# JuliaGaussianProcesses/AugmentedGPLikelihoods.jl

Measured on AMD Instinct MI355X. Metric: CAVI sweeps/sec (N obs, M inducing) + max |Δnat-param| vs CPU ref, higher is better.
Workload: dtype f32 via f16 hi/lo split operands (3 f16 MFMA products per f32 product, f32 accumulate, f64 reductions and M x M update)

## Files before the change

augmentedgplikelihoods.jl_amd/csrc/agpl_syrk.hip:

```cpp
#include <cstdlib>

#include "agpl_common.h"

namespace {

typedef _Float16 h8 __attribute__((ext_vector_type(8)));
typedef float f32x4 __attribute__((ext_vector_type(4)));
typedef unsigned u32x4 __attribute__((ext_vector_type(4)));

constexpr int BS = 128;
constexpr int kPanel = 256;
constexpr int kStagePts = 32;
constexpr uint32_t kImageMagic = 0x41474951u;

struct AccImageHeader {
    uint32_t magic;
    int32_t scale_exp;
    float max_abs;
    uint32_t reserved;
    int64_t N;
    int32_t M;
    int32_t pad[57];
};
static_assert(sizeof(AccImageHeader) == 256, "header size");

__device__ __forceinline__ f32x4 mfma32(h8 a, h8 b, f32x4 c) {
    return __builtin_amdgcn_mfma_f32_16x16x32_f16(a, b, c, 0, 0, 0);
}

#define AGPL_E_SPLIT2(x0_, s0_, x1_, s1_, H_, L_)                                                              \
    do {                                                                                                       \
        asm("v_fma_mixlo_f16 %0, %1, %2, 0" : "=v"(H_) : "v"(x0_), "v"(s0_));                                  \
        asm("v_fma_mixhi_f16 %0, %1, %2, 0" : "+v"(H_) : "v"(x1_), "v"(s1_));                                  \
        asm("v_fma_mixlo_f16 %0, %1, %2, -%3 op_sel_hi:[0,0,1]" : "=v"(L_) : "v"(x0_), "v"(s0_), "v"(H_));     \
        asm("v_fma_mixhi_f16 %0, %1, %2, -%3 op_sel:[0,0,1] op_sel_hi:[0,0,1]"                                 \
            : "+v"(L_)                                                                                         \
            : "v"(x1_), "v"(s1_), "v"(H_));                                                                    \
    } while (0)
#define AGPL_E_GFMA(acc_, b_, x_) asm volatile("v_fmac_f32 %0, %1, %2" : "+v"(acc_) : "v"(b_), "v"(x_))
#define AGPL_Q_JOIN2(H_, L_, x0_, x1_)                                                                         \
    do {                                                                                                       \
        asm("v_fma_mix_f32 %0, %1, 1.0, %2 op_sel_hi:[1,0,1]" : "=v"(x0_) : "v"(H_), "v"(L_));                 \
        asm("v_fma_mix_f32 %0, %1, 1.0, %2 op_sel:[1,0,1] op_sel_hi:[1,0,1]" : "=v"(x1_) : "v"(H_), "v"(L_));  \
    } while (0)

__global__ __launch_bounds__(256) void absmax_kernel(int64_t n4, int ntail, const float4 *__restrict__ x, unsigned *__restrict__ out) {
    unsigned m = 0u;
    for (int64_t i = (int64_t)blockIdx.x * blockDim.x + threadIdx.x; i < n4; i += (int64_t)gridDim.x * blockDim.x) {
        const float4 v = x[i];
        m = max(m, __float_as_uint(v.x) & 0x7FFFFFFFu);
        m = max(m, __float_as_uint(v.y) & 0x7FFFFFFFu);
        m = max(m, __float_as_uint(v.z) & 0x7FFFFFFFu);
        m = max(m, __float_as_uint(v.w) & 0x7FFFFFFFu);
    }
    if (blockIdx.x == 0 && (int)threadIdx.x < ntail)
        m = max(m, __float_as_uint(reinterpret_cast<const float *>(x)[4 * n4 + threadIdx.x]) & 0x7FFFFFFFu);
#pragma unroll
    for (int o = 32; o > 0; o >>= 1) m = max(m, (unsigned)__shfl_xor((int)m, o));
    if ((threadIdx.x & 63) == 0 && m) atomicMax(out, m);
}

__global__ __launch_bounds__(256) void find_bad_kernel(int64_t n, const float *__restrict__ x, float limit,
                                                       unsigned long long *__restrict__ out) {
    for (int64_t i = (int64_t)blockIdx.x * blockDim.x + threadIdx.x; i < n; i += (int64_t)gridDim.x * blockDim.x) {
        const float a = fabsf(x[i]);
        if (!(a < limit)) atomicMin(out, (unsigned long long)i);
    }
}

__global__ __launch_bounds__(256) void accumulate_image_kernel(int64_t N, int M, int Msrc, int64_t nps, float scale, int scale_exp,
                                                               float max_abs, const float *__restrict__ Phi,
                                                               unsigned char *__restrict__ image) {
    __shared__ float tile[16][BS + 1];
    const int nb = M / BS;
    if (blockIdx.x == 0 && threadIdx.x == 0) {
        AccImageHeader *h = reinterpret_cast<AccImageHeader *>(image);
        h->magic = kImageMagic;
        h->scale_exp = scale_exp;
        h->max_abs = max_abs;
        h->reserved = 0;
        h->N = N;
        h->M = M;
    }
    h8 *blocks = reinterpret_cast<h8 *>(image + sizeof(AccImageHeader));
    const int64_t nblk = nps * nb;
    for (int64_t blk = blockIdx.x; blk < nblk; blk += gridDim.x) {
        const int64_t ps = blk / nb;
        const int fb = (int)(blk - ps * nb);
        {
            const int pt = threadIdx.x >> 4, f0 = (threadIdx.x & 15) * 8;
            const int64_t n = ps * 16 + pt;
            float4 a = {0.f, 0.f, 0.f, 0.f}, b = a;
            if (n < N) {
                const int fg = fb * BS + f0;
                const float *src = Phi + n * (int64_t)Msrc + fg;
                if (!(Msrc & 3) && fg + 8 <= Msrc) {
                    a = *reinterpret_cast<const float4 *>(src);
                    b = *reinterpret_cast<const float4 *>(src + 4);
                } else {
                    float t[8];
#pragma unroll
                    for (int j = 0; j < 8; ++j) t[j] = fg + j < Msrc ? src[j] : 0.f;
                    a = float4{t[0], t[1], t[2], t[3]};
                    b = float4{t[4], t[5], t[6], t[7]};
                }
            }
            float *d = &tile[pt][f0];
            d[0] = a.x; d[1] = a.y; d[2] = a.z; d[3] = a.w;
            d[4] = b.x; d[5] = b.y; d[6] = b.z; d[7] = b.w;
        }
        __syncthreads();
        const int plane = threadIdx.x >> 7, row = threadIdx.x & 127;
        h8 hi, lo;
#pragma unroll
        for (int j = 0; j < 8; ++j) {
            const float x = tile[plane * 8 + j][row] * scale;
            const _Float16 a = (_Float16)x;
            hi[j] = a;
            lo[j] = (_Float16)(x - (float)a);
        }
        blocks[(blk * 2 + 0) * 256 + threadIdx.x] = hi;
        blocks[(blk * 2 + 1) * 256 + threadIdx.x] = lo;
        __syncthreads();
    }
}

__global__ __launch_bounds__(256) void acc_prep_kernel(int64_t N, int64_t Npad, int L, const float *__restrict__ gamma,
                                                        const float *__restrict__ beta, float *__restrict__ gb,
                                                        unsigned *__restrict__ scal) {
    __shared__ unsigned red[2][4];
    const int64_t total = (int64_t)L * Npad;
    unsigned m = 0u, bd = 0u;
    for (int64_t i = (int64_t)blockIdx.x * blockDim.x + threadIdx.x; i < total; i += (int64_t)gridDim.x * blockDim.x) {
        const int64_t l = i / Npad, n = i - l * Npad;
        const bool in = n < N;
        const float gv = in ? gamma[l * N + n] : 0.f;
        const unsigned gbits = __float_as_uint(gv), ab = gbits & 0x7FFFFFFFu;
        const bool bad = ab >= 0x7F800000u || ((gbits >> 31) && ab != 0u);
        if (bad) bd = max(bd, (unsigned)min((int64_t)0x7FFFFFFE, l * N + n) + 1u);
        m = max(m, bad ? 0u : ab);
        float *rec = gb + (l * (Npad / 32) + n / 32) * 64 + (n & 31);
        rec[0] = gv;
        rec[32] = in ? beta[l * N + n] : 0.f;
    }
#pragma unroll
    for (int o = 32; o > 0; o >>= 1) {
        m = max(m, (unsigned)__shfl_xor((int)m, o));
        bd = max(bd, (unsigned)__shfl_xor((int)bd, o));
    }
    if ((threadIdx.x & 63) == 0) {
        red[0][threadIdx.x >> 6] = m;
        red[1][threadIdx.x >> 6] = bd;
    }
    __syncthreads();
    if (threadIdx.x == 0) {
        for (int w = 1; w < 4; ++w) {
            m = max(m, red[0][w]);
            bd = max(bd, red[1][w]);
        }
        if (m) atomicMax(scal, m);
        if (bd) atomicMax(scal + 1, bd);
    }
}

__device__ __forceinline__ int acc_scale_exp(unsigned gmax) {
    int eB = gmax ? 126 - (int)(gmax >> 23) : 0;
    return eB < -60 ? -60 : (eB > 60 ? 60 : eB);
}

#ifdef AGPL_QTRACE
__device__ unsigned long long g_qtrace[64 * 16 * 8];
constexpr bool kTrace = true;
#else
constexpr bool kTrace = false;
#endif

#ifdef AGPL_SYRK_L2PROBE
#define AGPL_PROBE_T(t_) ((t_) & 3)
#else
#define AGPL_PROBE_T(t_) (t_)
#endif
#ifdef AGPL_SYRK_NODMA
#define AGPL_PROBE_LOAD(t_) ((t_) < 3)
#else
#define AGPL_PROBE_LOAD(t_) true
#endif
#ifndef AGPL_S_PRE
#define AGPL_S_PRE 3
#endif
constexpr int kStepBytes = 32768;
constexpr int kRing = 4;
constexpr int kRecBytes = 256;
constexpr int kStripLds = kRing * kStepBytes + 8 * kRing * kRecBytes;

template <bool DIAG>
__device__ __forceinline__ void syrk_strip_body(unsigned char *smem_raw, int64_t N, int64_t Npad, int M, int nsplit, int chunk, int nbig, int small, int l,
                                                int s, int I, int J, const unsigned char *__restrict__ image,
                                                const float *__restrict__ gb_all, const unsigned *__restrict__ scal,
                                                float *__restrict__ slabG, float *__restrict__ slabg) {
    typedef __attribute__((address_space(3))) void lds_void;
    const int lane = threadIdx.x & 63;
    const int wave = __builtin_amdgcn_readfirstlane(threadIdx.x >> 6);
    const int nb = M / BS;
    const int c = DIAG ? ((wave & 4) ? 7 - (wave & 3) : (wave & 3)) : wave;
    const int i0 = DIAG ? 2 * c : 0;
    const AccImageHeader *hdr = reinterpret_cast<const AccImageHeader *>(image);
    const h8 *blocks = reinterpret_cast<const h8 *>(image + sizeof(AccImageHeader));
    const int eA = hdr->scale_exp;
    const int eB = acc_scale_exp(scal[0]);
    const float sB = __uint_as_float((unsigned)(127 + eB) << 23);

    int64_t nbeg, nend;
    agpl_slice_range(s, chunk, nbig, small, N, nbeg, nend);
    const int nstep = (int)((nend - nbeg + kStagePts - 1) / kStagePts);
    const int64_t ps0 = nbeg / 16;
    const int64_t slice_pitch = (int64_t)nb * 2 * 256;

    int ln = lane;
    asm volatile("" : "+v"(ln));
    const int kg = ln >> 4, lr = ln & 15;
    const int rbS = (wave >> 2) & 1, qd = wave & 3;
    const h8 *a_src = blocks + ((ps0 * nb + 2 * I + rbS) * 2) * 256 + qd * 64 + lane;
    const int a_dst = rbS * 2 * 4096 + qd * 1024;
    const int R0 = 32 * c + lr;
    const h8 *b_src = blocks + (((ps0 + (kg >> 1)) * nb + 2 * J + (R0 >> 7)) * 2) * 256 + (kg & 1) * 128 + (R0 & 127);
    const float *gb_src = gb_all + ((int64_t)l * (Npad / 32) + nbeg / 32) * 64 + lane;
    float *gbuf = reinterpret_cast<float *>(smem_raw + kRing * kStepBytes + wave * kRing * kRecBytes);

    f32x4 acc[16][2];
#pragma unroll
    for (int i = 0; i < 16; ++i) acc[i][0] = acc[i][1] = f32x4{0.f, 0.f, 0.f, 0.f};
    float gacc0 = 0.f, gacc1 = 0.f;
    u32x4 rh0 = {0, 0, 0, 0}, rl0 = rh0, rh1 = rh0, rl1 = rh0;
    h8 bh0, bl0, bh1, bl1;

#define AGPL_S_DMA(t_, k_)                     \
    do {                                                                                                        \
        unsigned char *d_ = smem_raw + ((t_) & (kRing - 1)) * kStepBytes + ((k_) >> 1) * 16384 + a_dst + ((k_) & 1) * 4096; \
        const h8 *src_ = a_src + (int64_t)(2 * AGPL_PROBE_T(t_) + ((k_) >> 1)) * slice_pitch + ((k_) & 1) * 256; \
        if (AGPL_PROBE_LOAD(t_)) __builtin_amdgcn_global_load_lds(src_, (lds_void *)d_, 16, 0, 0);              \
    } while (0)
#define AGPL_S_DMAG(t_)                                                                                         \
    if (AGPL_PROBE_LOAD(t_))                                                                                    \
    __builtin_amdgcn_global_load_lds(gb_src + (int64_t)(t_) * 64, (lds_void *)(gbuf + ((t_) & (kRing - 1)) * 64), 4, 0, 0)
#define AGPL_S_LOADB(t_)                                                                                        \
    do {                                                                                                        \
        const h8 *src_ = b_src + (int64_t)(2 * AGPL_PROBE_T(t_)) * slice_pitch;                                 \
        const h8 *srcl_ = src_ + 256;  \
        if (AGPL_PROBE_LOAD(t_))                                                                                \
        asm volatile("global_load_dwordx4 %0, %4, off\n\tglobal_load_dwordx4 %1, %5, off\n\t"                   \
                     "global_load_dwordx4 %2, %4, off offset:256\n\tglobal_load_dwordx4 %3, %5, off offset:256"  \
                     : "+v"(rh0), "+v"(rl0), "+v"(rh1), "+v"(rl1)                                               \
                     : "v"(src_), "v"(srcl_)                                                                    \
                     : "memory");                                                                               \
    } while (0)
#define AGPL_S_CVT(RH_, RL_, g0_, g1_, b0_, b1_, GA_)                                                           \
    do {                                                                                                        \
        float x0_, x1_;                                                                                         \
        AGPL_Q_JOIN2(RH_, RL_, x0_, x1_);                                                                       \
        if (DIAG) {                                                                                             \
            AGPL_E_GFMA(GA_, b0_, x0_);                                                                         \
            AGPL_E_GFMA(GA_, b1_, x1_);                                                                         \
        }                                                                                                       \
        AGPL_E_SPLIT2(x0_, g0_, x1_, g1_, RH_, RL_);                                                            \
    } while (0)
#define AGPL_S_CVTQ(q_, tt_, keepf_)                                                                            \
    do {                                                                                                        \
        const float *gq_ = gbuf + ((tt_) & (kRing - 1)) * 64 + 8 * kg + 4 * ((q_) & 1);                         \
        float4 g4_ = *reinterpret_cast<const float4 *>(gq_);                                                    \
        g4_.x *= sB, g4_.y *= sB, g4_.z *= sB, g4_.w *= sB;                                                     \
        float4 b4_ = {0.f, 0.f, 0.f, 0.f};                                                                      \
        if (DIAG) {                                                                                             \
            b4_ = *reinterpret_cast<const float4 *>(gq_ + 32);                                                  \
            if (!(keepf_)) b4_ = float4{0.f, 0.f, 0.f, 0.f};                                                    \
        }                                                                                                       \
        if ((q_) == 0) {                                                                                        \
            AGPL_S_CVT(rh0.x, rl0.x, g4_.x, g4_.y, b4_.x, b4_.y, gacc0);                                        \
            AGPL_S_CVT(rh0.y, rl0.y, g4_.z, g4_.w, b4_.z, b4_.w, gacc0);                                        \
            AGPL_S_CVT(rh1.x, rl1.x, g4_.x, g4_.y, b4_.x, b4_.y, gacc1);                                        \
            AGPL_S_CVT(rh1.y, rl1.y, g4_.z, g4_.w, b4_.z, b4_.w, gacc1);                                        \
        } else {                                                                                                \
            AGPL_S_CVT(rh0.z, rl0.z, g4_.x, g4_.y, b4_.x, b4_.y, gacc0);                                        \
            AGPL_S_CVT(rh0.w, rl0.w, g4_.z, g4_.w, b4_.z, b4_.w, gacc0);                                        \
            AGPL_S_CVT(rh1.z, rl1.z, g4_.x, g4_.y, b4_.x, b4_.y, gacc1);                                        \
            AGPL_S_CVT(rh1.w, rl1.w, g4_.z, g4_.w, b4_.z, b4_.w, gacc1);                                        \
        }                                                                                                       \
    } while (0)
#define AGPL_S_TAKEB()                       \
    do {                                                                                                        \
        bh0 = __builtin_bit_cast(h8, rh0);                                                                      \
        bl0 = __builtin_bit_cast(h8, rl0);                                                                      \
        bh1 = __builtin_bit_cast(h8, rh1);                                                                      \
        bl1 = __builtin_bit_cast(h8, rl1);                                                                      \
    } while (0)

    const int fa = (kg >> 1) * 1024 + (kg & 1) * 128 + lr;
#define AGPL_S_AOFF(i_) (fa + ((i_) >> 3) * 512 + ((i_) & 7) * 16)
#define AGPL_S_LDSB(t_)                                                                                         \
    do {                                                                                                        \
        const u32x4 *sn_ = reinterpret_cast<const u32x4 *>(smem_raw + ((t_) & (kRing - 1)) * kStepBytes);       \
        rh0 = sn_[AGPL_S_AOFF(2 * c)];                                                                          \
        rl0 = sn_[256 + AGPL_S_AOFF(2 * c)];                                                                    \
        rh1 = sn_[AGPL_S_AOFF(2 * c + 1)];                                                                      \
        rl1 = sn_[256 + AGPL_S_AOFF(2 * c + 1)];                                                                \
    } while (0)

#pragma unroll
    for (int t = 0; t < 3; ++t)
        if (t < nstep) {
            AGPL_S_DMAG(t);
            AGPL_S_DMA(t, 0);
            AGPL_S_DMA(t, 1);
            AGPL_S_DMA(t, 2);
            AGPL_S_DMA(t, 3);
        }
    if (!DIAG) AGPL_S_LOADB(0);
    asm volatile("s_waitcnt vmcnt(0)" ::: "memory");
    __builtin_amdgcn_sched_barrier(0);
    if (DIAG) {
        __builtin_amdgcn_s_barrier();
        AGPL_S_LDSB(0);
    }
    AGPL_S_CVTQ(0, 0, true);
    AGPL_S_CVTQ(1, 0, true);
    AGPL_S_TAKEB();
    if (!DIAG) AGPL_S_LOADB(nstep > 1 ? 1 : 0);

    [[maybe_unused]] unsigned long long q0 = 0, q1 = 0, qw = 0, qa = 0, qb = 0, qr0 = 0;
    if (kTrace) {
        q0 = __builtin_amdgcn_s_memtime();
        qr0 = __builtin_amdgcn_s_memrealtime();
    }
    for (int t = 0; t < nstep; ++t) {
        if (kTrace) qa = __builtin_amdgcn_s_memtime();
        if (!DIAG) __builtin_amdgcn_s_barrier();
        if (kTrace && !DIAG) qw += __builtin_amdgcn_s_memtime() - qa;
        const bool more = t + 1 < nstep;
        const int tl = t + 2 < nstep ? t + 2 : nstep - 1;
        const h8 *st = reinterpret_cast<const h8 *>(smem_raw + (t & (kRing - 1)) * kStepBytes);
#define AGPL_S_HOOK(h_)                                                                                         \
    do {                                                                                                        \
        if (!DIAG) {                                                                                            \
            if ((h_) < 4 && t + 3 < nstep) {                                                                    \
                if ((h_) == 0) AGPL_S_DMAG(t + 3);                                                              \
                AGPL_S_DMA(t + 3, h_);                                                                          \
            }                                                                                                   \
            if ((h_) == 5) {  \
                __builtin_amdgcn_sched_barrier(0);                                                              \
                if (t + 3 < nstep) asm volatile("s_waitcnt vmcnt(5)" ::: "memory");                             \
                else asm volatile("s_waitcnt vmcnt(0)" ::: "memory");                                           \
                __builtin_amdgcn_sched_barrier(0);                                                              \
            }                                                                                                   \
            if ((h_) == 6) AGPL_S_CVTQ(0, t + 1, more);                                                         \
            if ((h_) == 8) AGPL_S_CVTQ(1, t + 1, more);                                                         \
        } else {                                                                                                \
             \
             \
             \
                 \
            if ((h_) == 7) {                                                                                    \
                __builtin_amdgcn_sched_barrier(0);                                                              \
                if (kTrace) qb = __builtin_amdgcn_s_memtime();                                                  \
                if (t + 2 < nstep) asm volatile("s_waitcnt vmcnt(5)" ::: "memory");                             \
                else asm volatile("s_waitcnt vmcnt(0)" ::: "memory");                                           \
                if (kTrace) q1 += __builtin_amdgcn_s_memtime() - qb;                                            \
                if (kTrace) qb = __builtin_amdgcn_s_memtime();                                                  \
                __builtin_amdgcn_s_barrier();                                                                   \
                if (kTrace) qw += __builtin_amdgcn_s_memtime() - qb;                                            \
                __builtin_amdgcn_sched_barrier(0);                                                              \
                AGPL_S_LDSB(more ? t + 1 : t);                 \
            }                                                                                                   \
            if ((h_) >= 8 && (h_) < 12 && t + 3 < nstep) {                                                      \
                if ((h_) == 8) AGPL_S_DMAG(t + 3);                                                              \
                AGPL_S_DMA(t + 3, (h_) - 8);                                                                    \
            }                                                                                                   \
            if ((h_) == 9) AGPL_S_CVTQ(0, t + 1, more);                                                         \
            if ((h_) == 11) AGPL_S_CVTQ(1, t + 1, more);                                                        \
        }                                                                                                       \
    } while (0)
        h8 nbh0, nbl0, nbh1, nbl1;
        constexpr int kPre = AGPL_S_PRE;
        h8 af[kPre + 1][2];
#pragma unroll
        for (int j = 0; j < kPre; ++j) {
            af[j][0] = st[AGPL_S_AOFF(j)];
            af[j][1] = st[256 + AGPL_S_AOFF(j)];
        }
#pragma unroll
        for (int i = 0; i < 16; ++i) {
            if (i + kPre < 16) {
                af[(i + kPre) % (kPre + 1)][0] = st[AGPL_S_AOFF(i + kPre)];
                af[(i + kPre) % (kPre + 1)][1] = st[256 + AGPL_S_AOFF(i + kPre)];
            }
            if (!DIAG || i >= i0) {
                const h8 ahc = af[i % (kPre + 1)][0], alc = af[i % (kPre + 1)][1];
                acc[i][0] = mfma32(ahc, bh0, acc[i][0]);
                acc[i][1] = mfma32(ahc, bh1, acc[i][1]);
                acc[i][0] = mfma32(ahc, bl0, acc[i][0]);
                acc[i][1] = mfma32(ahc, bl1, acc[i][1]);
                acc[i][0] = mfma32(alc, bh0, acc[i][0]);
                acc[i][1] = mfma32(alc, bh1, acc[i][1]);
            }
            AGPL_S_HOOK(i);
            if (i == (DIAG ? 12 : 10)) {
                nbh0 = __builtin_bit_cast(h8, rh0);
                nbl0 = __builtin_bit_cast(h8, rl0);
                nbh1 = __builtin_bit_cast(h8, rh1);
                nbl1 = __builtin_bit_cast(h8, rl1);
                if (!DIAG) AGPL_S_LOADB(tl);
            }
        }
#undef AGPL_S_HOOK
        bh0 = nbh0;
        bl0 = nbl0;
        bh1 = nbh1;
        bl1 = nbl1;
    }
#ifdef AGPL_QTRACE
    if (blockIdx.x < 64 && lane == 0) {
        unsigned long long *o = g_qtrace + ((size_t)blockIdx.x * 16 + wave) * 8;
        o[0] = q1;
        o[1] = __builtin_amdgcn_s_memtime() - q0;
        o[2] = qw;
        o[5] = __builtin_amdgcn_s_memrealtime() - qr0;
        o[6] = (unsigned long long)nstep | ((unsigned long long)(DIAG ? 1 : 0) << 32) | ((unsigned long long)c << 40);
        o[7] = o[1];
    }
#endif
    asm volatile("s_waitcnt vmcnt(0)" ::: "memory");
    asm volatile("" ::"v"(rh0), "v"(rl0), "v"(rh1), "v"(rl1));
#undef AGPL_S_DMA
#undef AGPL_S_DMAG
#undef AGPL_S_LOADB
#undef AGPL_S_CVT
#undef AGPL_S_CVTQ
#undef AGPL_S_TAKEB
#undef AGPL_S_LDSB
#undef AGPL_S_AOFF

    const float unscale = __uint_as_float((unsigned)(127 - (2 * eA + eB)) << 23);
    const int npairs = nb * (nb + 1) / 2;
    const int bj = 2 * J + (c >> 2);
#pragma unroll
    for (int hb = 0; hb < 2; ++hb) {
        const int bi = 2 * I + hb;
        if (DIAG && bi < bj) continue;
        const int p128 = bi * (bi + 1) / 2 + bj;
        float *slab = slabG + (((int64_t)l * npairs + p128) * nsplit + s) * (int64_t)(BS * BS);
#pragma unroll
        for (int ii = 0; ii < 8; ++ii)
#pragma unroll
            for (int cb = 0; cb < 2; ++cb)
#pragma unroll
                for (int r = 0; r < 4; ++r) {
                    const int row = 16 * ii + 4 * kg + r;
                    const int col = (c & 3) * 32 + 16 * cb + lr;
                    slab[row * BS + col] = acc[8 * hb + ii][cb][r] * unscale;
                }
    }
    if (DIAG) {
        gacc0 += __shfl_xor(gacc0, 16);
        gacc0 += __shfl_xor(gacc0, 32);
        gacc1 += __shfl_xor(gacc1, 16);
        gacc1 += __shfl_xor(gacc1, 32);
        const float g1s = __shfl(gacc1, (lane - 16) & 63);
        if (lane < 32) {
            const int rr = 32 * c + lane;
            slabg[(((int64_t)l * nb + 2 * I + (rr >> 7)) * nsplit + s) * BS + (rr & 127)] =
                (lane < 16 ? gacc0 : g1s) * __uint_as_float((unsigned)(127 - eA) << 23);
        }
    }
}


__global__ __launch_bounds__(512, 2) void syrk_strip_kernel(int64_t N, int64_t Npad, int M, int nlat, int npairs2, int nsplit, int chunk, int nbig, int small,
                                                            const unsigned char *__restrict__ image,
                                                            const float *__restrict__ gb_all,
                                                            const unsigned *__restrict__ scal,
                                                            float *__restrict__ slabG, float *__restrict__ slabg) {
    extern __shared__ __attribute__((aligned(16))) unsigned char smem_raw[];
    const int id = blockIdx.x;
    const int xcd = id & 7, jj = id >> 3;
    const int per_s = nlat * npairs2;
    const int s = (jj / per_s) * 8 + xcd;
    const int rem = jj % per_s;
    const int l = rem / npairs2;
    const int p2 = rem - l * npairs2;
    if (s >= nsplit) return;
    const int nb2 = M / kPanel;
    const int noff = nb2 * (nb2 - 1) / 2;
    int I, J;
    if (p2 < noff) {
        I = 1;
        while ((I + 1) * I / 2 <= p2) ++I;
        J = p2 - I * (I - 1) / 2;
    } else {
        I = J = p2 - noff;
    }
    if (I == J) syrk_strip_body<true>(smem_raw, N, Npad, M, nsplit, chunk, nbig, small, l, s, I, J, image, gb_all, scal, slabG, slabg);
    else syrk_strip_body<false>(smem_raw, N, Npad, M, nsplit, chunk, nbig, small, l, s, I, J, image, gb_all, scal, slabG, slabg);
}

}

#ifdef AGPL_QTRACE
extern "C" __attribute__((visibility("default"))) int agpl_debug_qtrace(unsigned long long *out) {
    return (int)hipMemcpyFromSymbol(out, HIP_SYMBOL(g_qtrace), sizeof(g_qtrace));
}
#endif


static_assert(sizeof(AccImageHeader) == 256 && BS == 128 && kStagePts == 32,
              "agpl_accumulate_image_bytes (agpl_common.h) assumes this layout");

int32_t agpl_feature_range_check(agpl_ctx *ctx, int64_t N, int32_t M, const float *Phi, float limit, const char *what,
                                 unsigned *max_bits_out) {
    int32_t rc = agpl_ws2_reserve(ctx, 4096);
    if (rc) return rc;
    if ((uintptr_t)Phi & 15) AGPL_FAIL(ctx, AGPL_ERR_INVALID_ARGUMENT, "the feature matrix must be 16-byte aligned");
    unsigned *mx = (unsigned *)ctx->ws2 + 512;
    AGPL_HIP(ctx, hipMemsetAsync(mx, 0, 16, ctx->stream));
    const int64_t n = N * (int64_t)M, n4 = n / 4;
    absmax_kernel<<<4096, 256, 0, ctx->stream>>>(n4, (int)(n - 4 * n4), reinterpret_cast<const float4 *>(Phi), mx);
    AGPL_LAUNCH_CHECK(ctx);
    unsigned hmx = 0, hlim;
    memcpy(&hlim, &limit, 4);
    AGPL_HIP(ctx, hipMemcpyAsync(&hmx, mx, sizeof(unsigned), hipMemcpyDeviceToHost, ctx->stream));
    AGPL_HIP(ctx, hipStreamSynchronize(ctx->stream));
    if (hmx >= 0x7F800000u || hmx >= hlim) {
        unsigned long long *bad = (unsigned long long *)(mx + 2), hbad = ~0ull;
        AGPL_HIP(ctx, hipMemsetAsync(bad, 0xFF, 8, ctx->stream));
        find_bad_kernel<<<4096, 256, 0, ctx->stream>>>(n, Phi, limit, bad);
        AGPL_HIP(ctx, hipMemcpyAsync(&hbad, bad, 8, hipMemcpyDeviceToHost, ctx->stream));
        AGPL_HIP(ctx, hipStreamSynchronize(ctx->stream));
        const long long pt = (long long)(hbad / (unsigned long long)M), ft = (long long)(hbad % (unsigned long long)M);
        if (hmx >= 0x7F800000u && !(limit < __builtin_inff()))
            AGPL_FAIL(ctx, AGPL_ERR_DOMAIN, "feature value is not finite (point %lld, feature %lld)", pt, ft);
        AGPL_FAIL(ctx, AGPL_ERR_DOMAIN,
                  "feature value is not finite or its magnitude is not below %g, the range of %s (point %lld, feature %lld)",
                  (double)limit, what, pt, ft);
    }
    *max_bits_out = hmx;
    return AGPL_OK;
}

int32_t agpl_image_scale_exp(agpl_ctx *ctx, unsigned hmx, int *eA_out) {
    int eA = 0;
    if (hmx) {
        const int ex = (int)(hmx >> 23) - 127;
        eA = 13 - ex;
        if (eA > 37 || eA < -30) {
            float mx;
            memcpy(&mx, &hmx, 4);
            AGPL_FAIL(ctx, AGPL_ERR_DOMAIN,
                      "max |Phi| = %g is outside the range the split-float16 images can be scaled for (2^-24 .. 2^44): rescale the "
                      "features", (double)mx);
        }
        if (eA > 30) eA = 30;
    }
    *eA_out = eA;
    return AGPL_OK;
}
int32_t agpl_accumulate_image_build(agpl_ctx *ctx, int64_t N, int32_t M, int32_t Msrc, const float *Phi, int eA, unsigned hmx,
                                    void *image_out) {
    float max_abs;
    memcpy(&max_abs, &hmx, 4);
    const float scale = ldexpf(1.f, eA);
    const int64_t nps = ((N + kStagePts - 1) / kStagePts) * 2;
    accumulate_image_kernel<<<16384, 256, 0, ctx->stream>>>(N, M, Msrc, nps, scale, eA, max_abs, Phi, (unsigned char *)image_out);
    AGPL_LAUNCH_CHECK(ctx);
    if (ctx->checked_image == image_out) ctx->checked_image = nullptr;
    return AGPL_OK;
}

int32_t agpl_syrk_image_launch(agpl_ctx *ctx, int64_t N, int64_t Npad, int32_t M, int32_t L, const void *image,
                               const float *gamma, const float *beta, float *gb, unsigned *scal, float *slabG,
                               float *slabg, int ns, int chunk, int nbig, int small, bool records_ready) {
    if (M % kPanel) AGPL_FAIL(ctx, AGPL_ERR_INVALID_ARGUMENT, "the image accumulation needs M %% 256 == 0 (M = %d)", M);
    if (ctx->checked_image != image || ctx->checked_image_N != N || ctx->checked_image_M != M) {
        AccImageHeader h;
        AGPL_HIP(ctx, hipMemcpyAsync(&h, image, sizeof(h), hipMemcpyDeviceToHost, ctx->stream));
        AGPL_HIP(ctx, hipStreamSynchronize(ctx->stream));
        if (h.magic != kImageMagic || h.N != N || h.M != M)
            AGPL_FAIL(ctx, AGPL_ERR_INVALID_ARGUMENT,
                      "not an accumulate image of this problem (agpl_plan_create): header says N = %lld, "
                      "M = %d, magic %#x; the call has N = %lld, M = %d",
                      (long long)h.N, (int)h.M, (unsigned)h.magic, (long long)N, (int)M);
        ctx->checked_image = image;
        ctx->checked_image_N = N;
        ctx->checked_image_M = M;
    }
    const int nb2 = M / kPanel;
    const int npairs2 = nb2 * (nb2 + 1) / 2;
    const int64_t nwg = (int64_t)L * npairs2 * ((ns + 7) / 8) * 8;
    if (nwg > 0x7fffffffLL) AGPL_FAIL(ctx, AGPL_ERR_INVALID_ARGUMENT, "problem too large for one launch");
    if (!records_ready) {
        AGPL_HIP(ctx, hipMemsetAsync(scal, 0, 2 * sizeof(unsigned), ctx->stream));
        int64_t nblk = agpl_cdiv((int64_t)L * Npad, 256);
        if (nblk > 1024) nblk = 1024;
        acc_prep_kernel<<<(unsigned)nblk, 256, 0, ctx->stream>>>(N, Npad, L, gamma, beta, gb, scal);
        AGPL_LAUNCH_CHECK(ctx);
    }
    if (!ctx->strip_attr) {
        AGPL_HIP(ctx, hipFuncSetAttribute(reinterpret_cast<const void *>(&syrk_strip_kernel),
                                          hipFuncAttributeMaxDynamicSharedMemorySize, kStripLds));
        ctx->strip_attr = 1;
    }
    syrk_strip_kernel<<<(unsigned)nwg, 512, kStripLds, ctx->stream>>>(N, Npad, M, L, npairs2, ns, chunk, nbig, small, (const unsigned char *)image, gb,
                                                                     scal, slabG, slabg);
    AGPL_LAUNCH_CHECK(ctx);
    return AGPL_OK;
}
```

Before: 75.63.

## Rebalance diagonal SYRK work with paired 16-column strips and stagger wave priorities

On diagonal tiles, each wave now owns two 16-column strips chosen as wave and 15-wave, so every wave gets a near-equal share of the lower-triangular MFMA work. Previously each wave owned one 32-column strip and skipped whole rows below its start, which left the waves with unequal loads. Off-diagonal tiles also gain s_setprio toggling, so the two halves of the workgroup take turns at higher priority across the MFMA loop and contend less. Epilogue indexing for slab and gradient writes is remapped to match, and a trace timer is added around the vmcnt wait.

```diff
diff --git a/augmentedgplikelihoods.jl_amd/csrc/agpl_syrk.hip b/augmentedgplikelihoods.jl_amd/csrc/agpl_syrk.hip
--- a/augmentedgplikelihoods.jl_amd/csrc/agpl_syrk.hip
+++ b/augmentedgplikelihoods.jl_amd/csrc/agpl_syrk.hip
@@ -202,8 +202,7 @@
     const int lane = threadIdx.x & 63;
     const int wave = __builtin_amdgcn_readfirstlane(threadIdx.x >> 6);
     const int nb = M / BS;
-    const int c = DIAG ? ((wave & 4) ? 7 - (wave & 3) : (wave & 3)) : wave;
-    const int i0 = DIAG ? 2 * c : 0;
+    const int cq0 = DIAG ? wave : 2 * wave, cq1 = DIAG ? 15 - wave : 2 * wave + 1;
     const AccImageHeader *hdr = reinterpret_cast<const AccImageHeader *>(image);
     const h8 *blocks = reinterpret_cast<const h8 *>(image + sizeof(AccImageHeader));
     const int eA = hdr->scale_exp;
@@ -222,7 +221,7 @@
     const int rbS = (wave >> 2) & 1, qd = wave & 3;
     const h8 *a_src = blocks + ((ps0 * nb + 2 * I + rbS) * 2) * 256 + qd * 64 + lane;
     const int a_dst = rbS * 2 * 4096 + qd * 1024;
-    const int R0 = 32 * c + lr;
+    const int R0 = 32 * wave + lr;
     const h8 *b_src = blocks + (((ps0 + (kg >> 1)) * nb + 2 * J + (R0 >> 7)) * 2) * 256 + (kg & 1) * 128 + (R0 & 127);
     const float *gb_src = gb_all + ((int64_t)l * (Npad / 32) + nbeg / 32) * 64 + lane;
     float *gbuf = reinterpret_cast<float *>(smem_raw + kRing * kStepBytes + wave * kRing * kRecBytes);
@@ -299,10 +298,10 @@
 #define AGPL_S_LDSB(t_)                                                                                         \
     do {                                                                                                        \
         const u32x4 *sn_ = reinterpret_cast<const u32x4 *>(smem_raw + ((t_) & (kRing - 1)) * kStepBytes);       \
-        rh0 = sn_[AGPL_S_AOFF(2 * c)];                                                                          \
-        rl0 = sn_[256 + AGPL_S_AOFF(2 * c)];                                                                    \
-        rh1 = sn_[AGPL_S_AOFF(2 * c + 1)];                                                                      \
-        rl1 = sn_[256 + AGPL_S_AOFF(2 * c + 1)];                                                                \
+        rh0 = sn_[AGPL_S_AOFF(cq0)];                                                                            \
+        rl0 = sn_[256 + AGPL_S_AOFF(cq0)];                                                                      \
+        rh1 = sn_[AGPL_S_AOFF(cq1)];                                                                            \
+        rl1 = sn_[256 + AGPL_S_AOFF(cq1)];                                                                      \
     } while (0)
 
 #pragma unroll
@@ -347,8 +346,10 @@
             }                                                                                                   \
             if ((h_) == 5) {  \
                 __builtin_amdgcn_sched_barrier(0);                                                              \
+                if (kTrace) qb = __builtin_amdgcn_s_memtime();                                                  \
                 if (t + 3 < nstep) asm volatile("s_waitcnt vmcnt(5)" ::: "memory");                             \
                 else asm volatile("s_waitcnt vmcnt(0)" ::: "memory");                                           \
+                if (kTrace) q1 += __builtin_amdgcn_s_memtime() - qb;                                            \
                 __builtin_amdgcn_sched_barrier(0);                                                              \
             }                                                                                                   \
             if ((h_) == 6) AGPL_S_CVTQ(0, t + 1, more);                                                         \
@@ -388,11 +389,15 @@
         }
 #pragma unroll
         for (int i = 0; i < 16; ++i) {
+            if (!DIAG && (i == 0 || i == 12)) {
+                if ((wave >= 4) == (i == 0)) __builtin_amdgcn_s_setprio(1);
+                else __builtin_amdgcn_s_setprio(0);
+            }
             if (i + kPre < 16) {
                 af[(i + kPre) % (kPre + 1)][0] = st[AGPL_S_AOFF(i + kPre)];
                 af[(i + kPre) % (kPre + 1)][1] = st[256 + AGPL_S_AOFF(i + kPre)];
             }
-            if (!DIAG || i >= i0) {
+            if (!DIAG) {
                 const h8 ahc = af[i % (kPre + 1)][0], alc = af[i % (kPre + 1)][1];
                 acc[i][0] = mfma32(ahc, bh0, acc[i][0]);
                 acc[i][1] = mfma32(ahc, bh1, acc[i][1]);
@@ -400,6 +405,18 @@
                 acc[i][1] = mfma32(ahc, bl1, acc[i][1]);
                 acc[i][0] = mfma32(alc, bh0, acc[i][0]);
                 acc[i][1] = mfma32(alc, bh1, acc[i][1]);
+            } else {
+                const h8 ahc = af[i % (kPre + 1)][0], alc = af[i % (kPre + 1)][1];
+                if (i >= cq0) {
+                    acc[i][0] = mfma32(ahc, bh0, acc[i][0]);
+                    acc[i][0] = mfma32(ahc, bl0, acc[i][0]);
+                    acc[i][0] = mfma32(alc, bh0, acc[i][0]);
+                }
+                if (i >= cq1) {
+                    acc[i][1] = mfma32(ahc, bh1, acc[i][1]);
+                    acc[i][1] = mfma32(ahc, bl1, acc[i][1]);
+                    acc[i][1] = mfma32(alc, bh1, acc[i][1]);
+                }
             }
             AGPL_S_HOOK(i);
             if (i == (DIAG ? 12 : 10)) {
@@ -416,6 +433,7 @@
         bh1 = nbh1;
         bl1 = nbl1;
     }
+    if (!DIAG) __builtin_amdgcn_s_setprio(0);
 #ifdef AGPL_QTRACE
     if (blockIdx.x < 64 && lane == 0) {
         unsigned long long *o = g_qtrace + ((size_t)blockIdx.x * 16 + wave) * 8;
@@ -423,7 +441,7 @@
         o[1] = __builtin_amdgcn_s_memtime() - q0;
         o[2] = qw;
         o[5] = __builtin_amdgcn_s_memrealtime() - qr0;
-        o[6] = (unsigned long long)nstep | ((unsigned long long)(DIAG ? 1 : 0) << 32) | ((unsigned long long)c << 40);
+        o[6] = (unsigned long long)nstep | ((unsigned long long)(DIAG ? 1 : 0) << 32) | ((unsigned long long)cq0 << 40);
         o[7] = o[1];
     }
 #endif
@@ -440,23 +458,25 @@
 
     const float unscale = __uint_as_float((unsigned)(127 - (2 * eA + eB)) << 23);
     const int npairs = nb * (nb + 1) / 2;
-    const int bj = 2 * J + (c >> 2);
 #pragma unroll
     for (int hb = 0; hb < 2; ++hb) {
         const int bi = 2 * I + hb;
-        if (DIAG && bi < bj) continue;
-        const int p128 = bi * (bi + 1) / 2 + bj;
-        float *slab = slabG + (((int64_t)l * npairs + p128) * nsplit + s) * (int64_t)(BS * BS);
-#pragma unroll
-        for (int ii = 0; ii < 8; ++ii)
-#pragma unroll
-            for (int cb = 0; cb < 2; ++cb)
+#pragma unroll
+        for (int cb = 0; cb < 2; ++cb) {
+            const int q = cb ? cq1 : cq0;
+            const int bj = 2 * J + (q >> 3);
+            if (DIAG && bi < bj) continue;
+            const int p128 = bi * (bi + 1) / 2 + bj;
+            float *slab = slabG + (((int64_t)l * npairs + p128) * nsplit + s) * (int64_t)(BS * BS);
+#pragma unroll
+            for (int ii = 0; ii < 8; ++ii)
 #pragma unroll
                 for (int r = 0; r < 4; ++r) {
                     const int row = 16 * ii + 4 * kg + r;
-                    const int col = (c & 3) * 32 + 16 * cb + lr;
+                    const int col = (q & 7) * 16 + lr;
                     slab[row * BS + col] = acc[8 * hb + ii][cb][r] * unscale;
                 }
+        }
     }
     if (DIAG) {
         gacc0 += __shfl_xor(gacc0, 16);
@@ -465,7 +485,7 @@
         gacc1 += __shfl_xor(gacc1, 32);
         const float g1s = __shfl(gacc1, (lane - 16) & 63);
         if (lane < 32) {
-            const int rr = 32 * c + lane;
+            const int rr = 16 * (lane < 16 ? cq0 : cq1) + (lane & 15);
             slabg[(((int64_t)l * nb + 2 * I + (rr >> 7)) * nsplit + s) * BS + (rr & 127)] =
                 (lane < 16 ? gacc0 : g1s) * __uint_as_float((unsigned)(127 - eA) << 23);
         }
```

Result: faster. 77.58 (median of 6 runs) (+2.6%).
